# Don-Yin/VAE-GAN

Measured on NVIDIA B200. Metric: train_images_per_sec, higher is better.
Workload: dtype bf16

## Files before the change

### include/vaegan_b200.h

```cpp
#ifndef VAEGAN_B200_H_
#define VAEGAN_B200_H_

#include <stddef.h>
#include <stdint.h>

#ifdef __cplusplus
extern "C" {
#endif

typedef void* vg_stream_t;

typedef enum {
  VG_OK = 0,
  VG_EINVAL = -1,
  VG_ECUDA = -2,
  VG_EARCH = -3,
  VG_EUNSUPPORTED = -4
} VgStatus;

typedef enum { VG_F32 = 0, VG_BF16 = 1 } VgDtype;

int vg_version(void);
int vg_init(int device);
const char* vg_last_error(void);
// ... 29 lines not shown
int vg_conv_dgrad(const VgConvDesc* d, const void* dy, const void* pack_kn, const void* pack_nk,
                  void* dx, vg_stream_t stream);
int vg_conv_forward_scaled(const VgConvDesc* d, const void* x, const void* pack_kn, const void* pack_nk,
                           const float* bias, const float* colscale, const float* sigma, int sigma_group_n,
                           void* y, double* stats, vg_stream_t stream);
int vg_conv_dgrad_scaled(const VgConvDesc* d, const void* dy, const void* pack_kn, const void* pack_nk,
                         const float* sigma, int sigma_group_n, void* dx, vg_stream_t stream);
typedef struct {
  const float* bias;
  const float* colscale;
  const float* sigma;
  int sigma_group_n;
  float act_slope;
  const void* residual;
  void* y2;
  const float* post_scale;
  const float* post_shift;
  float post_slope;
} VgConvEpilogue;
int vg_conv_forward_fused(const VgConvDesc* d, const void* x, const void* pack_kn, const void* pack_nk,
                          const VgConvEpilogue* ep, void* y, double* stats, vg_stream_t stream);
int vg_fold_bn_into_conv(const float* w, const float* bias_in, const float* gamma, const float* beta,
                         const float* running_mean, const float* running_var, float eps, int c_out, int c_in,
                         int inner, int transposed, float* w_out, float* bias_out, vg_stream_t stream);
int vg_bn_eval_affine(const float* gamma, const float* beta, const float* running_mean, const float* running_var,
                      float eps, int c, float* scale, float* shift, vg_stream_t stream);
int vg_conv_wgrad(const VgConvDesc* d, const void* x, const void* dy, float* dw, float* dbias,
                  float* workspace, vg_stream_t stream);

int vg_conv_tune_set(const VgConvDesc* d, int dgrad, int bn, int form);
int vg_conv_tune_clear(void);
int vg_conv_tune_record(int on);
int vg_conv_tune_seen(int* keys, int max_keys, int* count);

typedef struct {
  long long rows;
  int c;
  int hw;
  int dtype;
  float slope;
  float drop_p;
  unsigned long long seed;
  unsigned long long offset;
  long long sample_offset;
  int training;
  const unsigned long long* step_ptr;
} VgBnDesc;

int vg_bn_stats(const void* x, const VgBnDesc* d, double* sums, vg_stream_t stream);
int vg_bn_finalize(const double* sums, double count, int c, float eps, float momentum,
                   float* running_mean, float* running_var, float* mean_rstd, vg_stream_t stream);
int vg_bn_eval_stats(const float* running_mean, const float* running_var, int c, float eps,
                     float* mean_rstd, vg_stream_t stream);
int vg_bn_act_forward(const void* x, const float* mean_rstd, const float* gamma, const float* beta,
                      const VgBnDesc* d, void* y, vg_stream_t stream);
int vg_bn_act_backward_reduce(const void* dy, const void* x, const float* mean_rstd,
                              const float* gamma, const float* beta, const VgBnDesc* d,
                              double* sums, vg_stream_t stream);
int vg_bn_act_backward_apply(const void* dy, const void* x, const float* mean_rstd,
                             const float* gamma, const float* beta, const double* sums,
                             double count, const VgBnDesc* d, const float* out_colscale,
                             const void* addend, void* dx, vg_stream_t stream);
int vg_bn_param_grads(const double* sums, int c, float* dgamma, float* dbeta, vg_stream_t stream);

int vg_bn_add_forward(const void* a, const float* mean_rstd_a, const float* gamma_a,
                      const float* beta_a, const void* b, const float* mean_rstd_b,
// ... 145 lines not shown
```

### vae_gan_b200/_lib.py

```python
from __future__ import annotations

import ctypes as C
import os
from pathlib import Path

import torch

_PKG = Path(__file__).resolve().parent
LIB_PATH = Path(os.environ["VG_LIB"]) if os.environ.get("VG_LIB") else _PKG / "lib" / "libvaegan_sm100.so"

VG_F32, VG_BF16 = 0, 1

c_vp, c_int, c_ll, c_ull, c_f, c_d = C.c_void_p, C.c_int, C.c_longlong, C.c_ulonglong, C.c_float, C.c_double


class VgConvDesc(C.Structure):
    _fields_ = [(n, c_int) for n in ("n", "h_in", "w_in", "c_in", "h_out", "w_out", "c_out", "kh", "kw",
                                     "stride", "pad", "transposed", "act_dtype", "out_dtype")]


class VgBnDesc(C.Structure):
    _fields_ = [("rows", c_ll), ("c", c_int), ("hw", c_int), ("dtype", c_int), ("slope", c_f),
                ("drop_p", c_f), ("seed", c_ull), ("offset", c_ull), ("sample_offset", c_ll),
                ("training", c_int), ("step_ptr", c_vp)]
# ... 16 lines not shown
    _fields_ = [("bias", c_vp), ("colscale", c_vp), ("sigma", c_vp), ("sigma_group_n", c_int), ("act_slope", c_f),
                ("residual", c_vp), ("y2", c_vp), ("post_scale", c_vp), ("post_shift", c_vp), ("post_slope", c_f)]


class VgLossDesc(C.Structure):
    _fields_ = [("n_pix", c_ll), ("n_pix_global", c_ll), ("n_lat", c_ll), ("n_logits", c_int),
                ("n_logits_global", c_int), ("adv_mode", c_int), ("w_adv", c_f), ("w_recon", c_f),
                ("w_kl", c_f), ("xhat_dtype", c_int)]


class VgPeerDesc(C.Structure):
    _fields_ = [("peer_data", c_vp * 8), ("peer_flags", c_vp * 8), ("rank", c_int), ("world", c_int), ("n_slots", c_int)]


class VgOptDesc(C.Structure):
    _fields_ = [("kind", c_int), ("lr", c_f), ("beta1", c_f), ("beta2", c_f), ("alpha", c_f), ("eps", c_f),
                ("weight_decay", c_f), ("bias_corr1", c_f), ("bias_corr2", c_f), ("clamp", c_f),
                ("grad_scale", c_f)]


_PROTOS = {
    "vg_version": (c_int, []),
    "vg_init": (c_int, [c_int]),
    "vg_last_error": (C.c_char_p, []),
    "vg_launch_count": (c_ull, []),
    "vg_set_force_simt": (c_int, [c_int]),
    "vg_set_deterministic": (c_int, [c_int, c_vp, C.c_size_t, c_vp, c_int]),
    "vg_get_deterministic": (c_int, []),
    "vg_conv_pack_weights": (c_int, [C.POINTER(VgConvDesc), c_vp, c_vp, c_vp, c_vp, c_vp]),
    "vg_conv_wgrad_sn_supported": (c_int, [C.POINTER(VgConvDesc)]),
    "vg_conv_wgrad_sn": (c_int, [C.POINTER(VgConvDesc), c_vp, c_vp, c_vp, c_vp, c_vp, c_vp, c_vp, c_vp, c_vp, c_vp]),
    "vg_conv_tune_set": (c_int, [C.POINTER(VgConvDesc), c_int, c_int, c_int]),
    "vg_conv_tune_clear": (c_int, []),
    "vg_conv_tune_record": (c_int, [c_int]),
    "vg_conv_tune_seen": (c_int, [c_vp, c_int, C.POINTER(c_int)]),
    "vg_conv_pack_weights_batched": (c_int, [c_vp, c_int, c_int, c_vp]),
    "vg_conv_forward_scaled": (c_int, [C.POINTER(VgConvDesc), c_vp, c_vp, c_vp, c_vp, c_vp, c_vp, c_int, c_vp, c_vp, c_vp]),
    "vg_conv_forward_fused": (c_int, [C.POINTER(VgConvDesc), c_vp, c_vp, c_vp, C.POINTER(VgConvEpilogue), c_vp, c_vp, c_vp]),
    "vg_fold_bn_into_conv": (c_int, [c_vp, c_vp, c_vp, c_vp, c_vp, c_vp, c_f, c_int, c_int, c_int, c_int, c_vp, c_vp, c_vp]),
    "vg_bn_eval_affine": (c_int, [c_vp, c_vp, c_vp, c_vp, c_f, c_int, c_vp, c_vp, c_vp]),
    "vg_conv_dgrad_scaled": (c_int, [C.POINTER(VgConvDesc), c_vp, c_vp, c_vp, c_vp, c_int, c_vp, c_vp]),
    "vg_spectral_norm_sigma_batched": (c_int, [c_vp, c_int, c_int, c_f, c_vp, C.c_size_t, c_vp]),
    "vg_conv_forward": (c_int, [C.POINTER(VgConvDesc), c_vp, c_vp, c_vp, c_vp, c_vp, c_vp, c_vp, c_vp]),
    "vg_conv_dgrad": (c_int, [C.POINTER(VgConvDesc), c_vp, c_vp, c_vp, c_vp, c_vp]),
    "vg_conv_wgrad": (c_int, [C.POINTER(VgConvDesc), c_vp, c_vp, c_vp, c_vp, c_vp, c_vp]),
    "vg_bn_stats": (c_int, [c_vp, C.POINTER(VgBnDesc), c_vp, c_vp]),
    "vg_bn_finalize": (c_int, [c_vp, c_d, c_int, c_f, c_f, c_vp, c_vp, c_vp, c_vp]),
    "vg_bn_eval_stats": (c_int, [c_vp, c_vp, c_int, c_f, c_vp, c_vp]),
    "vg_bn_act_forward": (c_int, [c_vp, c_vp, c_vp, c_vp, C.POINTER(VgBnDesc), c_vp, c_vp]),
    "vg_bn_act_backward_reduce": (c_int, [c_vp, c_vp, c_vp, c_vp, c_vp, C.POINTER(VgBnDesc), c_vp, c_vp]),
    "vg_bn_act_backward_apply": (c_int, [c_vp, c_vp, c_vp, c_vp, c_vp, c_vp, c_d, C.POINTER(VgBnDesc), c_vp, c_vp, c_vp, c_vp]),
    "vg_bn_param_grads": (c_int, [c_vp, c_int, c_vp, c_vp, c_vp]),
    "vg_bn_add_forward": (c_int, [c_vp, c_vp, c_vp, c_vp, c_vp, c_vp, c_vp, c_vp, C.POINTER(VgBnDesc), c_vp, c_vp, c_vp]),
    "vg_bn_act_forward_fused": (c_int, [c_vp, C.POINTER(VgBnChannel), C.POINTER(VgBnDesc), c_vp, c_vp]),
    "vg_bn_add_forward_fused": (c_int, [c_vp, C.POINTER(VgBnChannel), c_vp, C.POINTER(VgBnChannel), C.POINTER(VgBnDesc), c_vp, c_vp, c_vp]),
    "vg_bn_act_backward_apply_fused": (c_int, [c_vp, c_vp, c_vp, c_vp, c_vp, c_vp, c_d, C.POINTER(VgBnDesc), c_vp, c_vp, c_vp,
                                               c_vp, c_vp, c_f, c_vp]),
    "vg_bn_param_grads_scaled": (c_int, [c_vp, c_int, c_f, c_vp, c_vp, c_vp]),
    "vg_add_dual_forward": (c_int, [c_vp, c_vp, c_vp, c_vp, c_f, C.POINTER(VgBnDesc), c_vp, c_vp, c_vp]),
    "vg_scale": (c_int, [c_vp, c_vp, c_ll, c_int, c_vp, c_vp]),
    "vg_normalize_images": (c_int, [c_vp, c_int, c_int, c_ll, c_vp, c_vp, c_vp]),
    "vg_lrelu_forward": (c_int, [c_vp, c_ll, c_int, c_f, c_vp, c_vp]),
    "vg_lrelu_backward": (c_int, [c_vp, c_vp, c_ll, c_int, c_f, c_vp, c_vp]),
    "vg_add": (c_int, [c_vp, c_vp, c_ll, c_int, c_vp, c_vp]),
    "vg_dropout_mask": (c_int, [C.POINTER(VgBnDesc), c_vp, c_vp]),
    "vg_dropout2d_scale": (c_int, [c_vp, c_int, c_int, c_f, c_ull, c_ull, c_vp, c_ll, c_vp]),
# ... 127 lines not shown
```

### vae_gan_b200/csrc/conv_api.cu

```cuda
#include "vg_common.cuh"

namespace vg {
int simt_conv_forward(const VgConvDesc*, const void*, const void*, const float*, const float*, const float* sigma, int sigma_group_n, void*,
                      cudaStream_t);
int simt_conv_dgrad(const VgConvDesc*, const void*, const void*, const float* sigma, int sigma_group_n, void*, cudaStream_t);
int simt_conv_wgrad(const VgConvDesc*, const void*, const void*, float*, cudaStream_t);
int simt_colsum(const void*, long long, int, int, float*, cudaStream_t);
int simt_pack_weights(const VgConvDesc*, const float*, const float*, void*, void*, cudaStream_t);
int simt_pack_weights_batched(const VgPackItem* items, int n_items, int dtype, cudaStream_t);
bool tc_conv_supported(const VgConvDesc*, bool dgrad);
bool tc_wgrad_supported(const VgConvDesc*);
int tc_conv_run(const VgConvDesc*, bool dgrad, const void* in, const void* wpack, const float* bias, const float* colscale,
                const float* sigma, int sigma_group_n, void* out, int out_dtype, cudaStream_t, const VgConvEpilogue* ep = nullptr);
int tc_wgrad_run(const VgConvDesc*, const void* x, const void* dy, float* dw, float* workspace, cudaStream_t, bool acc_only = false);
int sn_backward_run(const float* dw_hat, const float* w_orig, const float* u, const float* v, const float* sigma, int rows, int cols,
                    float* dw_orig, float* dot_ws, cudaStream_t s);
int sn_backward_packed_run(const float* acc, const float* w_orig, const float* u, const float* v, const float* sigma, int cu, int cs,
                           int taps, float* dw_orig, float* dot_ws, cudaStream_t s);
int simt_colsum(const void* x, long long rows, int c, int dtype, float* out, cudaStream_t s);
int tc_tune_set(const VgConvDesc*, int dgrad, int bn, int form);
void tc_tune_clear();
void tc_tune_record(int on);
int tc_tune_seen(int* keys, int max_keys);
}

using namespace vg;

static int check_conv(const VgConvDesc* d) {
  VG_CHECK_ARG(d != nullptr, "VgConvDesc is null");
  VG_CHECK_ARG(d->n >= 0 && d->h_in > 0 && d->w_in > 0 && d->c_in > 0 && d->c_out > 0, "bad conv dims");
  VG_CHECK_ARG(d->kh > 0 && d->kw > 0 && d->stride > 0 && d->pad >= 0, "bad conv kernel geometry");
  VG_CHECK_ARG(d->act_dtype == VG_F32 || d->act_dtype == VG_BF16, "bad act_dtype");
  VG_CHECK_ARG(d->out_dtype == VG_F32 || d->out_dtype == VG_BF16, "bad out_dtype");
  int eh, ew;
  if (d->transposed) {
    eh = (d->h_in - 1) * d->stride - 2 * d->pad + d->kh;
    ew = (d->w_in - 1) * d->stride - 2 * d->pad + d->kw;
  } else {
    eh = (d->h_in + 2 * d->pad - d->kh) / d->stride + 1;
    ew = (d->w_in + 2 * d->pad - d->kw) / d->stride + 1;
  }
  VG_CHECK_ARG(eh == d->h_out && ew == d->w_out, "output dims %dx%d inconsistent with geometry (expected %dx%d)", d->h_out, d->w_out, eh, ew);
  return VG_OK;
}

extern "C" int vg_conv_pack_weights(const VgConvDesc* d, const float* w, const float* sigma, void* pack_kn, void* pack_nk,
                                    vg_stream_t stream) {
  int rc = check_conv(d);
  if (rc) return rc;
  VG_CHECK_ARG(w && (pack_kn || pack_nk), "null pointer");
  return simt_pack_weights(d, w, sigma, pack_kn, pack_nk, as_stream(stream));
}

extern "C" int vg_conv_pack_weights_batched(const VgPackItem* items, int n_items, int dtype, vg_stream_t stream) {
  VG_CHECK_ARG(items != nullptr && n_items >= 0, "bad args");
  VG_CHECK_ARG(dtype == VG_F32 || dtype == VG_BF16, "bad dtype %d", dtype);
// ... 92 lines not shown
  if (d->n == 0) return VG_OK;
  VG_CHECK_ARG(x && dy && w_orig && u && v && sigma && dw_orig && workspace, "null pointer");
  if (!tc_wgrad_supported(d)) {
    set_error("vg_conv_wgrad_sn needs a tensor-core layer (bf16, channels %% 64 == 0): use vg_conv_wgrad + vg_spectral_norm_backward");
    return VG_EUNSUPPORTED;
  }
  cudaStream_t s = as_stream(stream);
  const int taps = d->kh * d->kw;
  const int cu = d->transposed ? d->c_in : d->c_out, cs = d->transposed ? d->c_out : d->c_in;
  const size_t welems = (size_t)taps * cu * cs;
  VG_CUDA(cudaMemsetAsync(workspace, 0, (welems + 4) * sizeof(float), s));
  if ((rc = tc_wgrad_run(d, x, dy, nullptr, workspace, s, true))) return rc;
  if (taps > 1) rc = sn_backward_packed_run(workspace, w_orig, u, v, sigma, cu, cs, taps, dw_orig, workspace + welems, s);
  else rc = sn_backward_run(workspace, w_orig, u, v, sigma, cu, cs, dw_orig, workspace + welems, s);
  if (rc) return rc;
  if (dbias) rc = simt_colsum(dy, (long long)d->n * d->h_out * d->w_out, d->c_out, d->act_dtype, dbias, s);
  return rc;
}

extern "C" int vg_conv_tune_set(const VgConvDesc* d, int dgrad, int bn, int form) { return vg::tc_tune_set(d, dgrad, bn, form); }
extern "C" int vg_conv_tune_clear(void) {
  vg::tc_tune_clear();
  return VG_OK;
}
extern "C" int vg_conv_tune_record(int on) {
  vg::tc_tune_record(on);
  return VG_OK;
}
extern "C" int vg_conv_tune_seen(int* keys, int max_keys, int* count) {
  VG_CHECK_ARG(count != nullptr && max_keys >= 0 && (keys != nullptr || max_keys == 0), "bad args");
  *count = vg::tc_tune_seen(keys, max_keys);
  return VG_OK;
}
```

### vae_gan_b200/csrc/conv_tc.cu

```cuda
#include <algorithm>
#include <array>
#include <map>
#include <mutex>
#include <vector>
#include "vg_common.cuh"
#include "sm100_ptx.cuh"

namespace vg {

struct TcTap {
  int8_t map, dy, dx, pad_;
  int32_t wrow;
};
struct TcPhase {
  int32_t ntaps, oy_off, ox_off, pad_;
  TcTap taps[16];
};
struct alignas(64) TcConvParams {
  CUtensorMap in_maps[4];
  CUtensorMap w_map;
  TcPhase phases[4];
  int tiles_x, tiles_y, tiles_n;
  int tw_log2, th_log2, TW, TH, TN;
  int gw, gh, gn;
  int k_chunks;
  int n_out;
  int n_store;
  int OH, OW, os;
  int out_f32;
  int ksplit, k_per_split;
  void* out;
  const float* bias;
  const float* colscale;
  const float* sigma;
  int sigma_group_n;
  float act_slope;
  const void* residual;
  void* out2;
  const float* post_scale;
  const float* post_shift;
  float post_slope;
  CUtensorMap out_maps[4];
  int tma_store;
  int* det_locks;
  long long det_split_stride;
};

struct alignas(64) TcWgradParams {
  CUtensorMap s_maps[4];
  CUtensorMap u_map;
  TcTap taps[16];
  int ntaps, cs_chunks, cs, cu;
  int tiles_x, tiles_y, tiles_n, TW, TH, TN;
  int n_boxes, boxes_per_split;
  int packed;
  float* dw;
  int* det_locks;
  long long det_split_stride;
};

constexpr int kTcThreads = 256;
constexpr int kABytes = 128 * 128;
constexpr int kStageBytes = 32 * 64;

template <int STAGES, int A_BYTES, int B_BYTES, int NACC, int EW>
struct TcSmem {
  static constexpr int kStages = STAGES, kA = A_BYTES, kB = B_BYTES;
  static constexpr int kBytes =
      1024 + STAGES * (A_BYTES + B_BYTES) + (2 * STAGES + NACC) * 8 + 16 + (EW > 0 ? 16 + 512 + EW * kStageBytes : 0);
  uint8_t* a;
  uint8_t* b;
  uint64_t* full;
  uint64_t* empty;
  uint64_t* acc;
  uint32_t* tmem_slot;
  uint8_t* stage;
  __device__ explicit TcSmem(uint8_t* raw) {
    a = raw + ((1024u - (ptx::smem_u32(raw) & 1023u)) & 1023u);
    b = a + STAGES * A_BYTES;
    full = reinterpret_cast<uint64_t*>(b + STAGES * B_BYTES);
    empty = full + STAGES;
    acc = empty + STAGES;
    tmem_slot = reinterpret_cast<uint32_t*>(acc + NACC);
    stage = reinterpret_cast<uint8_t*>((reinterpret_cast<uintptr_t>(tmem_slot + 4) + 511) & ~(uintptr_t)511);
  }
};

template <int BN, int STAGES>
using ConvSmem = TcSmem<STAGES, kABytes, BN * 128, 1, 4>;
template <int CTAS, int BN, int MT, int STAGES, int EW>
using ConvPersistSmem = TcSmem<STAGES, MT * kABytes, (BN / CTAS) * 128, 4, EW>;
template <int NB, int STAGES>
using WgradSmem = TcSmem<STAGES, (2 + NB) * 8192, 0, 1, 0>;

template <int CTAS, int TMEM_COLS, class Smem, class InitAcc>
__device__ __forceinline__ uint32_t tc_prologue(const Smem& sm, const CUtensorMap* map0, const CUtensorMap* map1, InitAcc init_acc) {
  const int warp = threadIdx.x >> 5, lane = threadIdx.x & 31;
  if (warp == 0 && lane == 0) {
    ptx::prefetch_tmap(map0);
    ptx::prefetch_tmap(map1);
  }
  if (warp == 1 && lane == 0) {
    for (int s = 0; s < Smem::kStages; ++s) {
      ptx::mbar_init(&sm.full[s], 1);
      ptx::mbar_init(&sm.empty[s], 1);
    }
    init_acc();
    ptx::fence_barrier_init();
  }
  if (warp == 2) {
    if constexpr (CTAS == 2) ptx::tmem_alloc_pair<TMEM_COLS>(sm.tmem_slot);
    else ptx::tmem_alloc<TMEM_COLS>(sm.tmem_slot);
  }
  ptx::tc_fence_before();
  if constexpr (CTAS == 2) ptx::cluster_sync();
  else __syncthreads();
  ptx::tc_fence_after();
  vg::pdl_entry();
  return *sm.tmem_slot;
}

template <int CTAS, int TMEM_COLS>
__device__ __forceinline__ void tc_teardown(uint32_t tmem_base) {
  ptx::tc_fence_before();
  if constexpr (CTAS == 2) ptx::cluster_sync();
  else __syncthreads();
// ... 426 lines not shown
        ptx::tc_fence_after();
      }
#pragma unroll 1
      for (int m = 0; m < nvalid; ++m)
        drain_tile<BN, EW, INF>(p, ph, e, tmem_base + (uint32_t)(as * kAccCols + m * BN), has_k, tile_origin(p, tile0 + m), true, nt * BN,
                                z, sm.stage);
      if (has_k) {
        ptx::tc_fence_before();
        __syncwarp();
        if (lane == 0) {
          if constexpr (CTAS == 2) ptx::mbar_arrive_cluster(ptx::mapa(ptx::smem_u32(&acc_empty[as]), 0));
          else ptx::mbar_arrive(&acc_empty[as]);
        }
        ++it;
      }
    }
    if (!INF && p.tma_store && lane == 0) ptx::bulk_wait_group0();
  }
  tc_teardown<CTAS, kTmemCols>(tmem_base);
}

template <int BN, int MT, int STAGES, int EW, bool INF>
__global__ void __launch_bounds__(128 + 32 * EW, 1)
    tc_conv_persist_kernel(const __grid_constant__ TcConvParams p, int n_ntiles, int n_groups, int n_work) {
  conv_persistent<1, BN, MT, STAGES, EW, INF>(p, n_ntiles, n_groups, n_work);
}

template <int BN, int MT, int STAGES, int EW, bool INF>
__global__ void __cluster_dims__(2, 1, 1) __launch_bounds__(128 + 32 * EW, 1)
    tc_conv_pair_kernel(const __grid_constant__ TcConvParams p, int n_ntiles, int n_groups, int n_work) {
  conv_persistent<2, BN, MT, STAGES, EW, INF>(p, n_ntiles, n_groups, n_work);
}

template <int NB, int STAGES>
__global__ void __launch_bounds__(kTcThreads) tc_wgrad_kernel(const __grid_constant__ TcWgradParams p) {
  using Smem = WgradSmem<NB, STAGES>;
  extern __shared__ uint8_t smem_raw[];
  constexpr int BN = NB * 64;
  constexpr int kStageBytes = Smem::kA;
  const Smem sm(smem_raw);
  uint8_t* const smem = sm.a;
  uint64_t* const full = sm.full;
  uint64_t* const empty = sm.empty;
  uint64_t* const tmem_full = sm.acc;

  const int warp = threadIdx.x >> 5, lane = threadIdx.x & 31;
  const int n_slabs = p.ntaps * p.cs_chunks;
  const int slab0 = blockIdx.x * 2;
  const bool has2 = slab0 + 1 < n_slabs;
  const int slab1 = has2 ? slab0 + 1 : slab0;
  const int box_begin = blockIdx.z * p.boxes_per_split;
  const int box_end = min(p.n_boxes, box_begin + p.boxes_per_split);
  const int num_k = max(0, box_end - box_begin);

  const uint32_t tmem_base = tc_prologue<1, BN>(sm, &p.u_map, &p.s_maps[0], [&] { ptx::mbar_init(tmem_full, 1); });

  if (num_k > 0) {
    if (warp == 0) {
      const int tapA = slab0 / p.cs_chunks, chA = slab0 % p.cs_chunks;
      const int tapB = slab1 / p.cs_chunks, chB = slab1 % p.cs_chunks;
      const TcTap ta = p.taps[tapA], tb = p.taps[tapB];
      int stage = 0;
      uint32_t phase = 0;
      for (int b = box_begin; b < box_end; ++b) {
        const Tile t = tile_origin(p, b);
        const int x0 = t.x0, y0 = t.y0, n0 = t.n0;
        ptx::mbar_wait(&empty[stage], phase ^ 1u);
        if (ptx::elect_one()) {
          ptx::mbar_arrive_expect_tx(&full[stage], kStageBytes);
          uint8_t* st = smem + stage * kStageBytes;
          ptx::tma_load_4d(st, &p.s_maps[ta.map], &full[stage], chA * 64, x0 + ta.dx, y0 + ta.dy, n0);
          ptx::tma_load_4d(st + 8192, &p.s_maps[tb.map], &full[stage], chB * 64, x0 + tb.dx, y0 + tb.dy, n0);
#pragma unroll
          for (int j = 0; j < NB; ++j)
            ptx::tma_load_4d(st + (2 + j) * 8192, &p.u_map, &full[stage], (blockIdx.y * NB + j) * 64, x0, y0, n0);
        }
        __syncwarp();
        if (++stage == STAGES) { stage = 0; phase ^= 1u; }
      }
    } else if (warp == 1) {
      constexpr uint32_t idesc = ptx::make_idesc_bf16(128, BN, 1, 1);
      constexpr uint32_t kDescHi = ptx::smem_desc_hi(1024);
      const uint32_t a_lo0 = ptx::smem_desc_lo(ptx::smem_u32(smem), 8192);
      uint32_t a_lo = a_lo0;
      int stage = 0;
      uint32_t phase = 0;
      for (int i = 0; i < num_k; ++i) {
        ptx::mbar_wait(&full[stage], phase);
        ptx::tc_fence_after();
        if (ptx::elect_one()) {
#pragma unroll
          for (int k = 0; k < 4; ++k)
            ptx::mma_bf16_ss_lohi(tmem_base, a_lo + (uint32_t)((k * 2048) >> 4), a_lo + (uint32_t)((2 * 8192 + k * 2048) >> 4), kDescHi,
                                  idesc, (i | k) != 0);
          ptx::mma_commit(&empty[stage]);
        }
        __syncwarp();
        if (++stage == STAGES) { stage = 0; phase ^= 1u; a_lo = a_lo0; }
        else a_lo += (uint32_t)(kStageBytes >> 4);
      }
      if (ptx::elect_one()) ptx::mma_commit(tmem_full);
      __syncwarp();
    }
  }

  int* const det_lock = p.det_locks != nullptr ? p.det_locks + (blockIdx.y * gridDim.x + blockIdx.x) : nullptr;
  if (warp >= 4 && det_lock) {
    if (lane == 0) det_wait_turn(det_lock, (int)blockIdx.z);
    __syncwarp();
  }
  if (warp >= 4 && num_k > 0) {
    const int q = warp - 4;
    const int row = q * 32 + lane;
    const int slab = (row < 64) ? slab0 : slab1;
    const bool row_valid = (row < 64) || has2;
    const int tap = slab / p.cs_chunks, chunk = slab % p.cs_chunks;
    const int cs = chunk * 64 + (row & 63);
    ptx::mbar_wait(tmem_full, 0);
    ptx::tc_fence_after();
#pragma unroll 1
    for (int c0 = 0; c0 < BN; c0 += 32) {
      uint32_t r[32];
      ptx::tmem_ld_32x32(tmem_base + ((uint32_t)(q * 32) << 16) + (uint32_t)c0, r);
      ptx::tmem_ld_wait();
      if (row_valid) {
        const int cu0 = blockIdx.y * BN + c0;
        if (p.packed) {
          float* dst = p.dw + (long long)blockIdx.z * p.det_split_stride + ((long long)tap * p.cs + cs) * p.cu + cu0;
          if (p.det_split_stride != 0) {
#pragma unroll
            for (int j = 0; j < 32; j += 4)
              *reinterpret_cast<float4*>(dst + j) = make_float4(__uint_as_float(r[j]), __uint_as_float(r[j + 1]), __uint_as_float(r[j + 2]),
                                                                __uint_as_float(r[j + 3]));
          } else {
#pragma unroll
            for (int j = 0; j < 32; j += 4)
              asm volatile("red.global.v4.f32.add [%0], {%1, %2, %3, %4};" ::"l"(dst + j), "f"(__uint_as_float(r[j])),
                           "f"(__uint_as_float(r[j + 1])), "f"(__uint_as_float(r[j + 2])), "f"(__uint_as_float(r[j + 3]))
                           : "memory");
          }
        } else {
#pragma unroll
          for (int j = 0; j < 32; ++j) {
            float* dst = p.dw + (long long)blockIdx.z * p.det_split_stride + ((long long)(cu0 + j) * p.cs + cs) * p.ntaps + tap;
            if (p.det_split_stride != 0) *dst = __uint_as_float(r[j]);
            else atomicAdd(dst, __uint_as_float(r[j]));
          }
        }
      }
    }
  }
  if (warp >= 4 && det_lock) {
    __threadfence();
    asm volatile("bar.sync 2, 128;" ::: "memory");
    if (warp == 4 && lane == 0) det_publish_turn(det_lock, blockIdx.z + 1 == gridDim.z ? 0 : (int)blockIdx.z + 1);
  }
  tc_teardown<1, BN>(tmem_base);
}

__global__ void __launch_bounds__(256) wgrad_unpack_kernel(const float* __restrict__ ws, int cu_n, int cs_n, int taps, float* __restrict__ dw) {
  vg::pdl_entry();
  __shared__ float tile[32][33];
  const int R = cs_n * taps;
  const int r0 = blockIdx.x * 32, c0 = blockIdx.y * 32;
  const int tx = threadIdx.x & 31, ty = threadIdx.x >> 5;
  for (int i = ty; i < 32; i += 8) {
    const int r = r0 + i, cu = c0 + tx;
    float v = 0.f;
    if (r < R && cu < cu_n) {
      const int cs = r / taps, tap = r - cs * taps;
      v = ws[((long long)tap * cs_n + cs) * cu_n + cu];
    }
    tile[i][tx] = v;
  }
  __syncthreads();
  for (int i = ty; i < 32; i += 8) {
    const int cu = c0 + i, r = r0 + tx;
    if (cu < cu_n && r < R) dw[(long long)cu * R + r] += tile[tx][i];
  }
}

typedef CUresult (*EncodeTiledFn)(CUtensorMap*, CUtensorMapDataType, cuuint32_t, void*, const cuuint64_t*, const cuuint64_t*,
                                  const cuuint32_t*, const cuuint32_t*, CUtensorMapInterleave, CUtensorMapSwizzle,
                                  CUtensorMapL2promotion, CUtensorMapFloatOOBfill);
static EncodeTiledFn g_encode = nullptr;
static std::once_flag g_encode_once;

static void bind_context_once() {
  static thread_local bool done = false;
  if (!done) {
// ... 303 lines not shown
  }
  static int tma_store = -1;
  if (tma_store < 0) { const char* e = getenv("VG_TC_TMA_STORE"); tma_store = e ? atoi(e) : 2; }
  if (tma_store && !p.out_f32 && p.ksplit == 1 && p.n_store != 1 && (p.os == 1 || tma_store >= 2) &&
      p.act_slope == 1.0f && p.residual == nullptr && p.out2 == nullptr) {
    const int bx = std::min(p.TW, 32), by = std::min(p.TH, 32 / bx), bn = 32 / (bx * by);
    for (int ph = 0; ph < nphase; ++ph)
      if ((rc = make_out_map(&p.out_maps[ph], out, d->n, out_h, out_w, n_out, bx, by, bn, p.os, p.phases[ph].oy_off, p.phases[ph].ox_off)))
        return rc;
    p.tma_store = 1;
  }
  const long long ctas1 = (long long)grid.x * grid.y * grid.z;
  const bool heur_persist = !(g_det.on && p.ksplit > 1) &&
                            ((BN == 256 && ctas1 > (long long)num_sms()) ||
                             (BN == 128 && ctas1 >= 2LL * num_sms()) ||
                             (BN == 64 && ctas1 >= (long long)kPersistMinItemsPerSm64 * num_sms()));
  const int form = p.ksplit > 1 ? kFormAuto : tuned.form;
  const bool use_persist = form == kFormAuto ? heur_persist : (form != kFormOneShot);
  int run_form = use_persist ? kFormPersist : kFormOneShot;
  if (use_persist && p.n_store != 1 && (form == kFormPair || (form == kFormAuto && BN >= kPairMinBN))) {
    const int mt = BN == 64 ? 4 : (BN == 128 ? 2 : 1);
    if (grid.x % (2 * mt) == 0) {
      if ((rc = make_weight_map(&p.w_map, wpack, (long long)k * k * n_out, in_c, BN / 2))) return rc;
      run_form = kFormPair;
    }
  }
  const bool inf = p.act_slope != 1.0f || p.residual != nullptr || p.out2 != nullptr;
  rc = inf ? launch_conv<true>(run_form, BN, p, grid, s) : launch_conv<false>(run_form, BN, p, grid, s);
  if (rc == VG_OK && p.det_split_stride != 0)
    rc = ordered_reduce_f32((const float*)p.out, p.ksplit, p.det_split_stride, (float*)out, s);
  return rc;
}

int tc_wgrad_run(const VgConvDesc* d, const void* x, const void* dy, float* dw, float* workspace, cudaStream_t s, bool acc_only) {
  TcWgradParams p;
  memset(&p, 0, sizeof(p));
  const void *U, *S;
  int hu, wu, cu, hs, ws, cs;
  if (!d->transposed) { U = dy; hu = d->h_out; wu = d->w_out; cu = d->c_out; S = x; hs = d->h_in; ws = d->w_in; cs = d->c_in; }
  else                { U = x;  hu = d->h_in;  wu = d->w_in;  cu = d->c_in;  S = dy; hs = d->h_out; ws = d->w_out; cs = d->c_out; }
  const int k = d->kh, st = d->stride, pad = d->pad;
  TcPhase tmp;
  build_gather_taps(&tmp, k, st, pad, 0);
  p.ntaps = tmp.ntaps;
  for (int i = 0; i < tmp.ntaps; ++i) p.taps[i] = tmp.taps[i];
  p.cs_chunks = cs / 64; p.cs = cs; p.cu = cu;
  choose_box(wu, hu, d->n, 64, &p.TW, &p.TH, &p.TN);
  p.tiles_x = (int)cdiv(wu, p.TW); p.tiles_y = (int)cdiv(hu, p.TH); p.tiles_n = (int)cdiv(d->n, p.TN);
  p.n_boxes = p.tiles_x * p.tiles_y * p.tiles_n;
  p.packed = workspace != nullptr && tmp.ntaps > 1;
  p.dw = (p.packed || acc_only) ? workspace : dw;
  const size_t welems = (size_t)k * k * cs * cu;
  if (p.packed && !acc_only) VG_CUDA(cudaMemsetAsync(workspace, 0, welems * sizeof(float), s));
  int rc;
  if (st == 2) {
    for (int py = 0; py < 2; ++py)
      for (int px = 0; px < 2; ++px)
        if ((rc = make_act_map(&p.s_maps[py * 2 + px], S, d->n, hs, ws, cs, 2, py, px, p.TW, p.TH, p.TN))) return rc;
  } else {
    if ((rc = make_act_map(&p.s_maps[0], S, d->n, hs, ws, cs, 1, 0, 0, p.TW, p.TH, p.TN))) return rc;
    p.s_maps[1] = p.s_maps[2] = p.s_maps[3] = p.s_maps[0];
  }
  if ((rc = make_act_map(&p.u_map, U, d->n, hu, wu, cu, 1, 0, 0, p.TW, p.TH, p.TN))) return rc;
  const int NB = (cu % 256 == 0) ? 4 : ((cu % 128 == 0) ? 2 : 1);
  const int m_tiles = (p.ntaps * p.cs_chunks + 1) / 2;
  const int n_tiles = cu / (NB * 64);
  if (p.n_boxes == 0) return VG_OK;
  const long long tiles = (long long)m_tiles * n_tiles;
  long long splits = 1;
  {
    double best = -1.0;
    const long long max_splits = std::max<long long>(1, p.n_boxes / 4);
    for (long long waves = 1; waves <= 4; ++waves) {
      long long sp = std::max<long long>(1, std::min<long long>((waves * num_sms()) / tiles, max_splits));
      long long bps = cdiv(p.n_boxes, sp);
      sp = cdiv(p.n_boxes, bps);
      const long long ctas = tiles * sp;
      const double eff = (double)ctas / (double)(cdiv(ctas, num_sms()) * num_sms());
      const double score = eff - 0.02 * (double)sp / (double)max_splits - (ctas < num_sms() ? 0.5 : 0.0);
      if (score > best) { best = score; splits = sp; }
    }
  }
  p.boxes_per_split = (int)cdiv(p.n_boxes, splits);
  splits = cdiv(p.n_boxes, p.boxes_per_split);
  dim3 grid((unsigned)m_tiles, (unsigned)n_tiles, (unsigned)splits);
  float* const wgrad_dst = p.dw;
  if (g_det.on && splits > 1) {
    if ((size_t)splits * welems * sizeof(float) <= g_det.scratch_bytes) {
      p.dw = (float*)g_det.scratch;
      p.det_split_stride = (long long)welems;
    } else if (!(p.det_locks = det_locks(tiles))) {
      return VG_EINVAL;
    }
  }
  switch (NB) {
    case 1: rc = launch<tc_wgrad_kernel<1, 6>>(grid, kTcThreads, WgradSmem<1, 6>::kBytes, s, p); break;
    case 2: rc = launch<tc_wgrad_kernel<2, 5>>(grid, kTcThreads, WgradSmem<2, 5>::kBytes, s, p); break;
    default: rc = launch<tc_wgrad_kernel<4, 4>>(grid, kTcThreads, WgradSmem<4, 4>::kBytes, s, p); break;
  }
  if (rc == VG_OK && p.det_split_stride != 0) rc = ordered_reduce_f32(p.dw, (int)splits, p.det_split_stride, wgrad_dst, s);
  if (rc || !p.packed || acc_only) return rc;
  dim3 ug((unsigned)cdiv((long long)cs * p.ntaps, 32), (unsigned)cdiv(cu, 32));
  vg::Launch(ug, 256, 0, s)(wgrad_unpack_kernel, workspace, cu, cs, p.ntaps, dw);
  VG_LAUNCHED();
  return VG_OK;
}

}
```

Baseline: 4410.

## Let wgrad CTAs own multiple slab pairs with halo-shared activation loads

```diff
diff --git a/include/vaegan_b200.h b/include/vaegan_b200.h
--- a/include/vaegan_b200.h
+++ b/include/vaegan_b200.h
@@ -85,6 +85,8 @@
 int vg_conv_tune_clear(void);
 int vg_conv_tune_record(int on);
 int vg_conv_tune_seen(int* keys, int max_keys, int* count);
+
+int vg_conv_wgrad_pin_slabs(int slabs_per_cta);
 
 typedef struct {
   long long rows;
diff --git a/vae_gan_b200/_lib.py b/vae_gan_b200/_lib.py
--- a/vae_gan_b200/_lib.py
+++ b/vae_gan_b200/_lib.py
@@ -72,6 +72,7 @@
     "vg_conv_wgrad_sn": (c_int, [C.POINTER(VgConvDesc), c_vp, c_vp, c_vp, c_vp, c_vp, c_vp, c_vp, c_vp, c_vp, c_vp]),
     "vg_conv_tune_set": (c_int, [C.POINTER(VgConvDesc), c_int, c_int, c_int]),
     "vg_conv_tune_clear": (c_int, []),
+    "vg_conv_wgrad_pin_slabs": (c_int, [c_int]),
     "vg_conv_tune_record": (c_int, [c_int]),
     "vg_conv_tune_seen": (c_int, [c_vp, c_int, C.POINTER(c_int)]),
     "vg_conv_pack_weights_batched": (c_int, [c_vp, c_int, c_int, c_vp]),
diff --git a/vae_gan_b200/csrc/conv_api.cu b/vae_gan_b200/csrc/conv_api.cu
--- a/vae_gan_b200/csrc/conv_api.cu
+++ b/vae_gan_b200/csrc/conv_api.cu
@@ -22,6 +22,7 @@
 void tc_tune_clear();
 void tc_tune_record(int on);
 int tc_tune_seen(int* keys, int max_keys);
+void tc_wgrad_pin_slabs(int slabs_per_cta);
 }
 
 using namespace vg;
@@ -180,3 +181,8 @@
   *count = vg::tc_tune_seen(keys, max_keys);
   return VG_OK;
 }
+extern "C" int vg_conv_wgrad_pin_slabs(int slabs_per_cta) {
+  VG_CHECK_ARG(slabs_per_cta >= 0, "slabs per CTA must be >= 0 (got %d)", slabs_per_cta);
+  vg::tc_wgrad_pin_slabs(slabs_per_cta);
+  return VG_OK;
+}
diff --git a/vae_gan_b200/csrc/conv_tc.cu b/vae_gan_b200/csrc/conv_tc.cu
--- a/vae_gan_b200/csrc/conv_tc.cu
+++ b/vae_gan_b200/csrc/conv_tc.cu
@@ -1,5 +1,6 @@
 #include <algorithm>
 #include <array>
+#include <atomic>
 #include <map>
 #include <mutex>
 #include <vector>
@@ -46,10 +47,21 @@
   long long det_split_stride;
 };
 
+struct TcWgradGroup {
+  int8_t map, dx, dy0, ntaps;
+  int32_t tap0;
+  int32_t slab0;
+  int32_t buf_bytes;
+};
+
 struct alignas(64) TcWgradParams {
   CUtensorMap s_maps[4];
   CUtensorMap u_map;
   TcTap taps[16];
+  TcWgradGroup groups[16];
+  int ngroups;
+  int slabs_per_cta;
+  int stage_bytes, stages;
   int ntaps, cs_chunks, cs, cu;
   int tiles_x, tiles_y, tiles_n, TW, TH, TN;
   int n_boxes, boxes_per_split;
@@ -90,8 +102,9 @@
 using ConvSmem = TcSmem<STAGES, kABytes, BN * 128, 1, 4>;
 template <int CTAS, int BN, int MT, int STAGES, int EW>
 using ConvPersistSmem = TcSmem<STAGES, MT * kABytes, (BN / CTAS) * 128, 4, EW>;
+constexpr int kWgradRingBytes = 192 * 1024;
 template <int NB, int STAGES>
-using WgradSmem = TcSmem<STAGES, (2 + NB) * 8192, 0, 1, 0>;
+using WgradSmem = TcSmem<STAGES, kWgradRingBytes / STAGES / 1024 * 1024, 0, 1, 0>;
 
 template <int CTAS, int TMEM_COLS, class Smem, class InitAcc>
 __device__ __forceinline__ uint32_t tc_prologue(const Smem& sm, const CUtensorMap* map0, const CUtensorMap* map1, InitAcc init_acc) {
@@ -584,12 +597,40 @@
   conv_persistent<2, BN, MT, STAGES, EW, INF>(p, n_ntiles, n_groups, n_work);
 }
 
+template <int MAX_SLABS, class F>
+__host__ __device__ __forceinline__ uint32_t walk_slabs(const TcWgradParams& p, int s_lo, int ns, F f) {
+  int g = 0;
+  while (g + 1 < p.ngroups && p.groups[g + 1].slab0 <= s_lo) ++g;
+  int j = s_lo - p.groups[g].slab0;
+  int c = j / p.groups[g].ntaps;
+  j -= c * p.groups[g].ntaps;
+  uint32_t buf = 0, next = 0;
+#pragma unroll
+  for (int i = 0; i < MAX_SLABS; ++i) {
+    if (i < ns) {
+      const TcWgradGroup& gr = p.groups[g];
+      const bool start = i == 0 || j == 0;
+      if (start) {
+        buf = next;
+        next += (uint32_t)gr.buf_bytes;
+      }
+      const TcTap& t = p.taps[gr.tap0 + j];
+      f(i, gr, t, c, start, buf, buf + (uint32_t)((t.dy - gr.dy0) * p.TW * 128));
+      if (++j == gr.ntaps) {
+        j = 0;
+        if (++c == p.cs_chunks) { c = 0; ++g; }
+      }
+    }
+  }
+  return next;
+}
+
 template <int NB, int STAGES>
-__global__ void __launch_bounds__(kTcThreads) tc_wgrad_kernel(const __grid_constant__ TcWgradParams p) {
+__global__ void __launch_bounds__(kTcThreads, 1) tc_wgrad_kernel(const __grid_constant__ TcWgradParams p) {
   using Smem = WgradSmem<NB, STAGES>;
   extern __shared__ uint8_t smem_raw[];
   constexpr int BN = NB * 64;
-  constexpr int kStageBytes = Smem::kA;
+  constexpr int kMaxAcc = 512 / BN, kMaxSlabs = 2 * kMaxAcc;
   const Smem sm(smem_raw);
   uint8_t* const smem = sm.a;
   uint64_t* const full = sm.full;
@@ -598,43 +639,59 @@
 
   const int warp = threadIdx.x >> 5, lane = threadIdx.x & 31;
   const int n_slabs = p.ntaps * p.cs_chunks;
-  const int slab0 = blockIdx.x * 2;
-  const bool has2 = slab0 + 1 < n_slabs;
-  const int slab1 = has2 ? slab0 + 1 : slab0;
+  const int s_lo = blockIdx.x * p.slabs_per_cta;
+  const int ns = min(p.slabs_per_cta, n_slabs - s_lo);
   const int box_begin = blockIdx.z * p.boxes_per_split;
   const int box_end = min(p.n_boxes, box_begin + p.boxes_per_split);
   const int num_k = max(0, box_end - box_begin);
 
-  const uint32_t tmem_base = tc_prologue<1, BN>(sm, &p.u_map, &p.s_maps[0], [&] { ptx::mbar_init(tmem_full, 1); });
+  const uint32_t tmem_base = tc_prologue<1, 512>(sm, &p.u_map, &p.s_maps[0], [&] { ptx::mbar_init(tmem_full, 1); });
 
   if (num_k > 0) {
     if (warp == 0) {
-      const int tapA = slab0 / p.cs_chunks, chA = slab0 % p.cs_chunks;
-      const int tapB = slab1 / p.cs_chunks, chB = slab1 % p.cs_chunks;
-      const TcTap ta = p.taps[tapA], tb = p.taps[tapB];
+      uint32_t boff[kMaxSlabs], bch[kMaxSlabs], bsh[kMaxSlabs];
+      const uint32_t x_bytes = walk_slabs<kMaxSlabs>(p, s_lo, ns, [&](int i, const TcWgradGroup& gr, const TcTap&, int c, bool start,
+                                                                       uint32_t buf, uint32_t) {
+        boff[i] = start ? buf : ~0u;
+        bch[i] = (uint32_t)c * 64;
+        bsh[i] = (uint32_t)gr.map | ((uint32_t)(uint8_t)gr.dx << 8) | ((uint32_t)(uint8_t)gr.dy0 << 16);
+      });
       int stage = 0;
       uint32_t phase = 0;
       for (int b = box_begin; b < box_end; ++b) {
         const Tile t = tile_origin(p, b);
-        const int x0 = t.x0, y0 = t.y0, n0 = t.n0;
         ptx::mbar_wait(&empty[stage], phase ^ 1u);
         if (ptx::elect_one()) {
-          ptx::mbar_arrive_expect_tx(&full[stage], kStageBytes);
-          uint8_t* st = smem + stage * kStageBytes;
-          ptx::tma_load_4d(st, &p.s_maps[ta.map], &full[stage], chA * 64, x0 + ta.dx, y0 + ta.dy, n0);
-          ptx::tma_load_4d(st + 8192, &p.s_maps[tb.map], &full[stage], chB * 64, x0 + tb.dx, y0 + tb.dy, n0);
+          ptx::mbar_arrive_expect_tx(&full[stage], x_bytes + NB * 8192);
+          uint8_t* st = smem + stage * p.stage_bytes;
+#pragma unroll
+          for (int i = 0; i < kMaxSlabs; ++i)
+            if (i < ns && boff[i] != ~0u)
+              ptx::tma_load_4d(st + boff[i], &p.s_maps[bsh[i] & 3u], &full[stage], (int)bch[i], t.x0 + (int8_t)(bsh[i] >> 8),
+                               t.y0 + (int8_t)(bsh[i] >> 16), t.n0);
 #pragma unroll
           for (int j = 0; j < NB; ++j)
-            ptx::tma_load_4d(st + (2 + j) * 8192, &p.u_map, &full[stage], (blockIdx.y * NB + j) * 64, x0, y0, n0);
+            ptx::tma_load_4d(st + x_bytes + j * 8192, &p.u_map, &full[stage], (blockIdx.y * NB + j) * 64, t.x0, t.y0, t.n0);
         }
         __syncwarp();
-        if (++stage == STAGES) { stage = 0; phase ^= 1u; }
+        if (++stage == p.stages) { stage = 0; phase ^= 1u; }
       }
     } else if (warp == 1) {
       constexpr uint32_t idesc = ptx::make_idesc_bf16(128, BN, 1, 1);
       constexpr uint32_t kDescHi = ptx::smem_desc_hi(1024);
-      const uint32_t a_lo0 = ptx::smem_desc_lo(ptx::smem_u32(smem), 8192);
-      uint32_t a_lo = a_lo0;
+      uint32_t soff[kMaxSlabs];
+      const uint32_t x_bytes = walk_slabs<kMaxSlabs>(p, s_lo, ns, [&](int i, const TcWgradGroup&, const TcTap&, int, bool, uint32_t,
+                                                                       uint32_t off) { soff[i] = off; });
+      uint32_t a_rel[kMaxAcc];
+#pragma unroll
+      for (int a = 0; a < kMaxAcc; ++a) {
+        const uint32_t lo = soff[2 * a], hi = 2 * a + 1 < ns ? soff[2 * a + 1] : x_bytes;
+        a_rel[a] = (lo >> 4) | (((hi - lo) >> 4) << 16);
+      }
+      const uint32_t b_rel = (x_bytes >> 4) | ((8192u >> 4) << 16);
+      const int nacc = (ns + 1) / 2;
+      const uint32_t base0 = ptx::smem_u32(smem) >> 4;
+      uint32_t base = base0;
       int stage = 0;
       uint32_t phase = 0;
       for (int i = 0; i < num_k; ++i) {
@@ -642,14 +699,18 @@
         ptx::tc_fence_after();
         if (ptx::elect_one()) {
 #pragma unroll
-          for (int k = 0; k < 4; ++k)
-            ptx::mma_bf16_ss_lohi(tmem_base, a_lo + (uint32_t)((k * 2048) >> 4), a_lo + (uint32_t)((2 * 8192 + k * 2048) >> 4), kDescHi,
-                                  idesc, (i | k) != 0);
+          for (int a = 0; a < kMaxAcc; ++a)
+            if (a < nacc) {
+#pragma unroll
+              for (int k = 0; k < 4; ++k)
+                ptx::mma_bf16_ss_lohi(tmem_base + (uint32_t)(a * BN), base + a_rel[a] + (uint32_t)(k * 128), base + b_rel + (uint32_t)(k * 128),
+                                      kDescHi, idesc, (i | k) != 0);
+            }
           ptx::mma_commit(&empty[stage]);
         }
         __syncwarp();
-        if (++stage == STAGES) { stage = 0; phase ^= 1u; a_lo = a_lo0; }
-        else a_lo += (uint32_t)(kStageBytes >> 4);
+        if (++stage == p.stages) { stage = 0; phase ^= 1u; base = base0; }
+        else base += (uint32_t)(p.stage_bytes >> 4);
       }
       if (ptx::elect_one()) ptx::mma_commit(tmem_full);
       __syncwarp();
@@ -664,39 +725,47 @@
   if (warp >= 4 && num_k > 0) {
     const int q = warp - 4;
     const int row = q * 32 + lane;
-    const int slab = (row < 64) ? slab0 : slab1;
-    const bool row_valid = (row < 64) || has2;
-    const int tap = slab / p.cs_chunks, chunk = slab % p.cs_chunks;
-    const int cs = chunk * 64 + (row & 63);
+    const int half = row >> 6;
+    uint32_t slab_tc[kMaxSlabs];
+    walk_slabs<kMaxSlabs>(p, s_lo, ns, [&](int i, const TcWgradGroup&, const TcTap& t, int c, bool, uint32_t, uint32_t) {
+      slab_tc[i] = ((uint32_t)t.wrow << 16) | (uint32_t)c;
+    });
     ptx::mbar_wait(tmem_full, 0);
     ptx::tc_fence_after();
+#pragma unroll
+    for (int a = 0; a < kMaxAcc; ++a) {
+      if (2 * a >= ns) break;
+      const bool row_valid = 2 * a + half < ns;
+      const uint32_t tc = half ? (2 * a + 1 < ns ? slab_tc[2 * a + 1] : 0u) : slab_tc[2 * a];
+      const int tap = (int)(tc >> 16), cs = (int)(tc & 0xffffu) * 64 + (row & 63);
 #pragma unroll 1
-    for (int c0 = 0; c0 < BN; c0 += 32) {
-      uint32_t r[32];
-      ptx::tmem_ld_32x32(tmem_base + ((uint32_t)(q * 32) << 16) + (uint32_t)c0, r);
-      ptx::tmem_ld_wait();
-      if (row_valid) {
-        const int cu0 = blockIdx.y * BN + c0;
-        if (p.packed) {
-          float* dst = p.dw + (long long)blockIdx.z * p.det_split_stride + ((long long)tap * p.cs + cs) * p.cu + cu0;
-          if (p.det_split_stride != 0) {
-#pragma unroll
-            for (int j = 0; j < 32; j += 4)
-              *reinterpret_cast<float4*>(dst + j) = make_float4(__uint_as_float(r[j]), __uint_as_float(r[j + 1]), __uint_as_float(r[j + 2]),
-                                                                __uint_as_float(r[j + 3]));
+      for (int c0 = 0; c0 < BN; c0 += 32) {
+        uint32_t r[32];
+        ptx::tmem_ld_32x32(tmem_base + ((uint32_t)(q * 32) << 16) + (uint32_t)(a * BN + c0), r);
+        ptx::tmem_ld_wait();
+        if (row_valid) {
+          const int cu0 = blockIdx.y * BN + c0;
+          if (p.packed) {
+            float* dst = p.dw + (long long)blockIdx.z * p.det_split_stride + ((long long)tap * p.cs + cs) * p.cu + cu0;
+            if (p.det_split_stride != 0) {
+#pragma unroll
+              for (int j = 0; j < 32; j += 4)
+                *reinterpret_cast<float4*>(dst + j) = make_float4(__uint_as_float(r[j]), __uint_as_float(r[j + 1]), __uint_as_float(r[j + 2]),
+                                                                  __uint_as_float(r[j + 3]));
+            } else {
+#pragma unroll
+              for (int j = 0; j < 32; j += 4)
+                asm volatile("red.global.v4.f32.add [%0], {%1, %2, %3, %4};" ::"l"(dst + j), "f"(__uint_as_float(r[j])),
+                             "f"(__uint_as_float(r[j + 1])), "f"(__uint_as_float(r[j + 2])), "f"(__uint_as_float(r[j + 3]))
+                             : "memory");
+            }
           } else {
 #pragma unroll
-            for (int j = 0; j < 32; j += 4)
-              asm volatile("red.global.v4.f32.add [%0], {%1, %2, %3, %4};" ::"l"(dst + j), "f"(__uint_as_float(r[j])),
-                           "f"(__uint_as_float(r[j + 1])), "f"(__uint_as_float(r[j + 2])), "f"(__uint_as_float(r[j + 3]))
-                           : "memory");
-          }
-        } else {
-#pragma unroll
-          for (int j = 0; j < 32; ++j) {
-            float* dst = p.dw + (long long)blockIdx.z * p.det_split_stride + ((long long)(cu0 + j) * p.cs + cs) * p.ntaps + tap;
-            if (p.det_split_stride != 0) *dst = __uint_as_float(r[j]);
-            else atomicAdd(dst, __uint_as_float(r[j]));
+            for (int j = 0; j < 32; ++j) {
+              float* dst = p.dw + (long long)blockIdx.z * p.det_split_stride + ((long long)(cu0 + j) * p.cs + cs) * p.ntaps + tap;
+              if (p.det_split_stride != 0) *dst = __uint_as_float(r[j]);
+              else atomicAdd(dst, __uint_as_float(r[j]));
+            }
           }
         }
       }
@@ -707,7 +776,7 @@
     asm volatile("bar.sync 2, 128;" ::: "memory");
     if (warp == 4 && lane == 0) det_publish_turn(det_lock, blockIdx.z + 1 == gridDim.z ? 0 : (int)blockIdx.z + 1);
   }
-  tc_teardown<1, BN>(tmem_base);
+  tc_teardown<1, 512>(tmem_base);
 }
 
 __global__ void __launch_bounds__(256) wgrad_unpack_kernel(const float* __restrict__ ws, int cu_n, int cs_n, int taps, float* __restrict__ dw) {
@@ -1077,6 +1146,9 @@
   return rc;
 }
 
+static std::atomic<int> g_wgrad_pin_slabs{0};
+void tc_wgrad_pin_slabs(int slabs_per_cta) { g_wgrad_pin_slabs.store(slabs_per_cta); }
+
 int tc_wgrad_run(const VgConvDesc* d, const void* x, const void* dy, float* dw, float* workspace, cudaStream_t s, bool acc_only) {
   TcWgradParams p;
   memset(&p, 0, sizeof(p));
@@ -1085,14 +1157,40 @@
   if (!d->transposed) { U = dy; hu = d->h_out; wu = d->w_out; cu = d->c_out; S = x; hs = d->h_in; ws = d->w_in; cs = d->c_in; }
   else                { U = x;  hu = d->h_in;  wu = d->w_in;  cu = d->c_in;  S = dy; hs = d->h_out; ws = d->w_out; cs = d->c_out; }
   const int k = d->kh, st = d->stride, pad = d->pad;
-  TcPhase tmp;
-  build_gather_taps(&tmp, k, st, pad, 0);
-  p.ntaps = tmp.ntaps;
-  for (int i = 0; i < tmp.ntaps; ++i) p.taps[i] = tmp.taps[i];
   p.cs_chunks = cs / 64; p.cs = cs; p.cu = cu;
   choose_box(wu, hu, d->n, 64, &p.TW, &p.TH, &p.TN);
   p.tiles_x = (int)cdiv(wu, p.TW); p.tiles_y = (int)cdiv(hu, p.TH); p.tiles_n = (int)cdiv(d->n, p.TN);
   p.n_boxes = p.tiles_x * p.tiles_y * p.tiles_n;
+  TcPhase tmp;
+  build_gather_taps(&tmp, k, st, pad, 1);
+  p.ntaps = tmp.ntaps;
+  const bool halo = p.TN == 1 && p.TW >= 8;
+  int rows[4] = {p.TH, p.TH, p.TH, p.TH};
+  {
+    bool used[16] = {};
+    int nt = 0;
+    for (int i = 0; i < tmp.ntaps; ++i) {
+      if (used[i]) continue;
+      TcWgradGroup& g = p.groups[p.ngroups++];
+      g.map = tmp.taps[i].map; g.dx = tmp.taps[i].dx; g.tap0 = nt; g.ntaps = 0;
+      for (int j = i; j < tmp.ntaps; ++j)
+        if (j == i || (halo && !used[j] && tmp.taps[j].map == g.map && tmp.taps[j].dx == g.dx)) {
+          used[j] = true;
+          p.taps[nt++] = tmp.taps[j];
+          ++g.ntaps;
+        }
+      std::sort(p.taps + g.tap0, p.taps + nt, [](const TcTap& a, const TcTap& b) { return a.dy < b.dy; });
+      g.dy0 = p.taps[g.tap0].dy;
+      rows[g.map] = std::max(rows[g.map], p.TH + p.taps[nt - 1].dy - g.dy0);
+    }
+    int slab = 0;
+    for (int i = 0; i < p.ngroups; ++i) {
+      TcWgradGroup& g = p.groups[i];
+      g.slab0 = slab;
+      slab += g.ntaps * p.cs_chunks;
+      g.buf_bytes = p.TW * rows[g.map] * p.TN * 128;
+    }
+  }
   p.packed = workspace != nullptr && tmp.ntaps > 1;
   p.dw = (p.packed || acc_only) ? workspace : dw;
   const size_t welems = (size_t)k * k * cs * cu;
@@ -1101,31 +1199,75 @@
   if (st == 2) {
     for (int py = 0; py < 2; ++py)
       for (int px = 0; px < 2; ++px)
-        if ((rc = make_act_map(&p.s_maps[py * 2 + px], S, d->n, hs, ws, cs, 2, py, px, p.TW, p.TH, p.TN))) return rc;
+        if ((rc = make_act_map(&p.s_maps[py * 2 + px], S, d->n, hs, ws, cs, 2, py, px, p.TW, rows[py * 2 + px], p.TN))) return rc;
   } else {
-    if ((rc = make_act_map(&p.s_maps[0], S, d->n, hs, ws, cs, 1, 0, 0, p.TW, p.TH, p.TN))) return rc;
+    if ((rc = make_act_map(&p.s_maps[0], S, d->n, hs, ws, cs, 1, 0, 0, p.TW, rows[0], p.TN))) return rc;
     p.s_maps[1] = p.s_maps[2] = p.s_maps[3] = p.s_maps[0];
   }
   if ((rc = make_act_map(&p.u_map, U, d->n, hu, wu, cu, 1, 0, 0, p.TW, p.TH, p.TN))) return rc;
   const int NB = (cu % 256 == 0) ? 4 : ((cu % 128 == 0) ? 2 : 1);
-  const int m_tiles = (p.ntaps * p.cs_chunks + 1) / 2;
   const int n_tiles = cu / (NB * 64);
   if (p.n_boxes == 0) return VG_OK;
+  const int n_slabs = p.ntaps * p.cs_chunks;
+  const int max_stages = NB == 1 ? 6 : (NB == 2 ? 5 : 4);
+  const int ring = NB == 1 ? WgradSmem<1, 6>::kStages * WgradSmem<1, 6>::kA
+                           : (NB == 2 ? WgradSmem<2, 5>::kStages * WgradSmem<2, 5>::kA : WgradSmem<4, 4>::kStages * WgradSmem<4, 4>::kA);
+  long long splits = 1;
+  int m_tiles = 1;
+  {
+    const int BN = NB * 64;
+    const double mma_cycles = 4.0 * std::max(BN / 2.0, 32.0 + BN / 4.0);
+    const double red_cycles_per_split = (double)welems * sizeof(float) / 380.0;
+    const long long max_splits = std::max<long long>(1, p.n_boxes / 4);
+    long long det_splits = 0;
+    if (g_det.on) {
+      const long long tiles2 = cdiv(n_slabs, 2) * (long long)n_tiles;
+      double best_score = -1.0;
+      for (long long waves = 1; waves <= 4; ++waves) {
+        long long sp = std::max<long long>(1, std::min<long long>((waves * num_sms()) / tiles2, max_splits));
+        sp = cdiv(p.n_boxes, cdiv(p.n_boxes, sp));
+        const long long ctas = tiles2 * sp;
+        const double eff = (double)ctas / (double)(cdiv(ctas, num_sms()) * num_sms());
+        const double score = eff - 0.02 * (double)sp / (double)max_splits - (ctas < num_sms() ? 0.5 : 0.0);
+        if (score > best_score) { best_score = score; det_splits = sp; }
+      }
+    }
+    const int max_spc = 2 * (512 / BN);
+    const int pin = std::min(max_spc, (g_wgrad_pin_slabs.load() + 1) & ~1);
+    double best = 1e300;
+    int best_spc = 2, best_bytes = 0;
+    for (int pass = pin > 0 ? 0 : 1; pass < 2 && best_bytes == 0; ++pass) {
+      for (int spc = 2; spc <= max_spc; spc += 2) {
+        if (pass == 0 && spc != pin) continue;
+        p.slabs_per_cta = spc;
+        int max_bytes = 0;
+        double box_cycles = 0.0;
+        for (int s0 = 0; s0 < n_slabs; s0 += spc) {
+          const int ns = std::min(spc, n_slabs - s0);
+          const int bytes = (int)walk_slabs<16>(p, s0, ns, [](int, const TcWgradGroup&, const TcTap&, int, bool, uint32_t, uint32_t) {}) +
+                            NB * 8192;
+          max_bytes = std::max(max_bytes, bytes);
+          box_cycles = std::max(box_cycles, std::max(mma_cycles * ((ns + 1) / 2), bytes / 64.0));
+        }
+        if (ring / max_bytes >= (pass == 0 || spc == 2 ? 2 : 3)) {
+          const long long tiles = cdiv(n_slabs, spc) * (long long)n_tiles;
+          for (long long waves = 1; waves <= (det_splits > 0 ? 1 : 4); ++waves) {
+            long long sp = det_splits > 0 ? det_splits : std::max<long long>(1, std::min<long long>((waves * num_sms()) / tiles, max_splits));
+            const long long bps = cdiv(p.n_boxes, sp);
+            sp = cdiv(p.n_boxes, bps);
+            const double t = (double)cdiv(tiles * sp, num_sms()) * (double)bps * box_cycles + (double)sp * red_cycles_per_split;
+            if (t < best) { best = t; best_spc = spc; best_bytes = max_bytes; splits = sp; }
+          }
+        }
+        if (spc >= n_slabs && pass == 1) break;
+      }
+    }
+    p.slabs_per_cta = best_spc;
+    p.stage_bytes = best_bytes;
+    p.stages = std::min(max_stages, ring / best_bytes);
+    m_tiles = (int)cdiv(n_slabs, best_spc);
+  }
   const long long tiles = (long long)m_tiles * n_tiles;
-  long long splits = 1;
-  {
-    double best = -1.0;
-    const long long max_splits = std::max<long long>(1, p.n_boxes / 4);
-    for (long long waves = 1; waves <= 4; ++waves) {
-      long long sp = std::max<long long>(1, std::min<long long>((waves * num_sms()) / tiles, max_splits));
-      long long bps = cdiv(p.n_boxes, sp);
-      sp = cdiv(p.n_boxes, bps);
-      const long long ctas = tiles * sp;
-      const double eff = (double)ctas / (double)(cdiv(ctas, num_sms()) * num_sms());
-      const double score = eff - 0.02 * (double)sp / (double)max_splits - (ctas < num_sms() ? 0.5 : 0.0);
-      if (score > best) { best = score; splits = sp; }
-    }
-  }
   p.boxes_per_split = (int)cdiv(p.n_boxes, splits);
   splits = cdiv(p.n_boxes, p.boxes_per_split);
   dim3 grid((unsigned)m_tiles, (unsigned)n_tiles, (unsigned)splits);
```

Measured after the change: 4521 (median of 6 runs). 2.5% higher.
